# tijiang13/InstantAvatar

Hardware: AMD Instinct MI355X
Metric: novel_pose_render_frames_per_sec_512x512 (higher is better)
Workload: dtype f32; 1 GPU; render_image_fast 512x512, SNARF_NGP defaults (13 init bones, 128^2x32 skinning voxels, 16-level hash grid T=2^19, 64^3 occupancy rebuilt per frame with 5 probes, MAX_SAMPLES 256, MAX_BATCH 291600), synthetic SMPL-like body animated by the first 200 frames of data/animation/aist_demo.npz (animate.py:48-50 translation; tests/golden/aist_demo_200.npz); pose_track=aist_demo.npz[:200]

## Files before the change

### instantavatar_amd/csrc/ia_render.hip

```cpp
#include "ia_common.h"

int ia_launch_field(const float *x, int V, const int32_t *n_dev, const FieldDev &F, float *rgb,
                    float *sigma, hipStream_t s, uint16_t *acts);

__device__ __forceinline__ float clampf(float f, float a, float b) { return fmaxf(a, fminf(f, b)); }

__device__ __forceinline__ bool occ_test(const uint32_t *__restrict__ bits, int G, int nx, int ny, int nz) {
  const uint32_t idx = (uint32_t)((nx * G + ny) * G + nz);
  return (bits[idx >> 5] >> (idx & 31)) & 1u;
}

struct MarchRay {
  float ox, oy, oz, dx, dy, dz, cx, cy, cz, sx, sy, sz, far, dt;
};

__device__ __forceinline__ bool march_occupied(const MarchRay &r, const uint32_t *__restrict__ bits, int G,
                                               float t, float &x, float &y, float &z) {
  x = __builtin_fmaf(t, r.dx, r.ox); y = __builtin_fmaf(t, r.dy, r.oy); z = __builtin_fmaf(t, r.dz, r.oz);
  const float fx = (x - r.cx) * r.sx, fy = (y - r.cy) * r.sy, fz = (z - r.cz) * r.sz;
  const int nx = (int)clampf(fx, 0.0f, G - 1.0f);
  const int ny = (int)clampf(fy, 0.0f, G - 1.0f);
  const int nz = (int)clampf(fz, 0.0f, G - 1.0f);
  return occ_test(bits, G, nx, ny, nz);
}

__device__ __forceinline__ void march_skip(float &t, float dt, float lim) {
  if (dt > 0.f) {
    for (;;) {
      const float a = t + dt, b = a + dt, c = b + dt, d = c + dt, e = d + dt, f = e + dt, g = f + dt;
      if (!(g < lim)) break;
      t = g + dt;
    }
  }
  while (t < lim) t += dt;
}

__device__ __forceinline__ MarchRay load_ray(const float *__restrict__ o, const float *__restrict__ d,
                                             const float *__restrict__ fars, const float *__restrict__ step,
                                             size_t n, const float *aabb_mn, const float *aabb_mx, int G) {
  MarchRay r;
  r.ox = o[n * 3]; r.oy = o[n * 3 + 1]; r.oz = o[n * 3 + 2];
  r.dx = d[n * 3]; r.dy = d[n * 3 + 1]; r.dz = d[n * 3 + 2];
  r.cx = aabb_mn[0]; r.cy = aabb_mn[1]; r.cz = aabb_mn[2];
  r.sx = G / (aabb_mx[0] - aabb_mn[0]); r.sy = G / (aabb_mx[1] - aabb_mn[1]); r.sz = G / (aabb_mx[2] - aabb_mn[2]);
  r.far = fars[n]; r.dt = step[n];
  return r;
}

__global__ __launch_bounds__(256) void k_raymarch_test(const float *__restrict__ rays_o,
                                                       const float *__restrict__ rays_d, float *nears,
                                                       const float *__restrict__ fars,
                                                       const int64_t *__restrict__ alive, int n_alive,
                                                       const uint32_t *__restrict__ bits, OccDev occ,
                                                       const float *__restrict__ step, int N_steps,
                                                       float *__restrict__ pts, float *__restrict__ deltas,
                                                       float *__restrict__ depths) {
  const int i = blockIdx.x * blockDim.x + threadIdx.x;
  if (i >= n_alive) return;
  const size_t n = (size_t)alive[i];
  const MarchRay r = load_ray(rays_o, rays_d, fars, step, n, occ.mn, occ.mx, occ.G);
  int s = 0;
  float t = nears[n];
  while (t < r.far && s < N_steps) {
    float x, y, z;
    if (march_occupied(r, bits, occ.G, t, x, y, z)) {
      const size_t o = (size_t)i * N_steps + s;
      pts[o * 3] = x; pts[o * 3 + 1] = y; pts[o * 3 + 2] = z;
      deltas[o] = r.dt; depths[o] = t;
      s++;
    }
    t += r.dt;
  }
  for (; s < N_steps; s++) {
    const size_t o = (size_t)i * N_steps + s;
    pts[o * 3] = 0.f; pts[o * 3 + 1] = 0.f; pts[o * 3 + 2] = 0.f;
    deltas[o] = 0.f; depths[o] = 0.f;
  }
  nears[n] = t;
}

__global__ __launch_bounds__(256) void k_raymarch_train(const float *__restrict__ rays_o,
                                                        const float *__restrict__ rays_d,
                                                        const float *__restrict__ nears,
                                                        const float *__restrict__ fars, int n_rays,
                                                        const uint32_t *__restrict__ bits, OccDev occ,
                                                        const float *__restrict__ step, int N_steps,
                                                        float *__restrict__ depths) {
  const int n = blockIdx.x * blockDim.x + threadIdx.x;
  if (n >= n_rays) return;
  const MarchRay r = load_ray(rays_o, rays_d, fars, step, (size_t)n, occ.mn, occ.mx, occ.G);
  int s = 0;
  float t = nears[n];
  while (t < r.far && s < N_steps) {
    float x, y, z;
    if (march_occupied(r, bits, occ.G, t, x, y, z)) { depths[(size_t)n * N_steps + s] = t; s++; }
    t += r.dt;
  }
  for (; s < N_steps; s++) depths[(size_t)n * N_steps + s] = 0.f;
}

__device__ __forceinline__ void composite_step(float sg, float dl, float tdepth, const float *rgb3,
                                               float thresh, float &T, float &c0, float &c1, float &c2,
                                               float &dep) {
  const float tau = __expf(-sg * dl);
  const float alpha = 1.0f - tau;
  if (alpha < thresh) return;
  const float w = alpha * T;
  c0 += w * rgb3[0]; c1 += w * rgb3[1]; c2 += w * rgb3[2];
  dep += w * tdepth;
  T *= tau;
}

__global__ __launch_bounds__(256) void k_composite_test(const float *__restrict__ rgb,
                                                        const float *__restrict__ sigma,
                                                        const float *__restrict__ delta,
                                                        const float *__restrict__ depth,
                                                        const int64_t *__restrict__ alive, int n_alive,
                                                        int N_steps, float *color, float *depth_out,
                                                        float *nohit, float thresh) {
  const int i = blockIdx.x * blockDim.x + threadIdx.x;
  if (i >= n_alive) return;
  const size_t n = (size_t)alive[i];
  float T = nohit[n];
  float c0 = color[n * 3], c1 = color[n * 3 + 1], c2 = color[n * 3 + 2], dep = depth_out[n];
  int s = 0;
  while (s < N_steps && (double)T > 1e-4 && delta[(size_t)i * N_steps + s] > 0) {
    const size_t o = (size_t)i * N_steps + s;
    composite_step(sigma[o], delta[o], depth[o], rgb + o * 3, thresh, T, c0, c1, c2, dep);
    s++;
  }
  color[n * 3] = c0; color[n * 3 + 1] = c1; color[n * 3 + 2] = c2;
  depth_out[n] = dep;
  nohit[n] = T;
}

__device__ __forceinline__ void cand_max(const float *__restrict__ cand_rgb,
                                         const float *__restrict__ cand_sigma, int off, int cnt, int n_init,
                                         float fill, bool nan_to_num, float &sg, float *rgb3) {
  float best;
  int bi = -1;
  rgb3[0] = rgb3[1] = rgb3[2] = 0.f;
  if (cnt < n_init) best = fill; else best = -INFINITY;
  for (int c = 0; c < cnt; c++) {
    float s = cand_sigma[off + c];
    if (nan_to_num && !isfinite(s)) s = 0.f;
    if (s > best || (bi < 0 && cnt >= n_init && c == 0)) { best = s; bi = c; }
  }
  if (bi >= 0) {
#pragma unroll
    for (int k = 0; k < 3; k++) {
      float v = cand_rgb[(size_t)(off + bi) * 3 + k];
      if (nan_to_num && !isfinite(v)) v = 0.f;
      rgb3[k] = v;
    }
  }
  sg = best;
}

__global__ __launch_bounds__(256) void k_candidate_max(const float *__restrict__ cand_rgb,
                                                       const float *__restrict__ cand_sigma,
                                                       const int32_t *__restrict__ pt_off,
                                                       const uint8_t *__restrict__ pt_cnt, int P,
                                                       const int32_t *__restrict__ n_pts_dev, int n_init,
                                                       float fill, int nan_to_num, float *__restrict__ rgb,
                                                       float *__restrict__ sigma, float *__restrict__ dmax) {
  if (n_pts_dev) P = min(P, *n_pts_dev);
  const int p = blockIdx.x * blockDim.x + threadIdx.x;
  if (p >= P) return;
  float sg, c[3];
  cand_max(cand_rgb, cand_sigma, pt_off[p], pt_cnt[p], n_init, fill, nan_to_num != 0, sg, c);
  if (sigma) sigma[p] = sg;
  if (rgb) { rgb[(size_t)p * 3] = c[0]; rgb[(size_t)p * 3 + 1] = c[1]; rgb[(size_t)p * 3 + 2] = c[2]; }
  if (dmax) dmax[p] = fmaxf(dmax[p], sg);
}

struct OccWs {
  double sum;
  unsigned long long best;
  float thr;
  float pad;
};

__global__ __launch_bounds__(256) void k_occ_pool(const float *__restrict__ density, int G,
                                                  float *__restrict__ pooled, double *__restrict__ partial,
                                                  int32_t *__restrict__ parent, int32_t *__restrict__ count,
                                                  OccWs *__restrict__ ws, uint32_t *__restrict__ bits) {
  const int n = G * G * G;
  const int i = blockIdx.x * blockDim.x + threadIdx.x;
  if (i == 0) { ws->sum = 0.0; ws->best = 0ull; bits[n >> 5] = 1u; }
  float m = 0.f;
  if (i < n) {
    const int x = i / (G * G), y = i / G % G, z = i % G;
    m = -INFINITY;
    for (int a = -1; a <= 1; a++)
      for (int b = -1; b <= 1; b++)
        for (int c = -1; c <= 1; c++) {
          const int xx = x + a, yy = y + b, zz = z + c;
          if (xx < 0 || yy < 0 || zz < 0 || xx >= G || yy >= G || zz >= G) continue;
          const float f = 1.f - expf(0.01f * -density[(xx * G + yy) * G + zz]);
          m = (f > m || isnan(f)) ? f : m;
        }
    pooled[i] = m;
    parent[i] = i;
    count[i] = 0;
  }
  __shared__ double s_part[4];
  double v = (i < n) ? (double)m : 0.0;
#pragma unroll
  for (int o = 32; o > 0; o >>= 1) v += __shfl_xor(v, o, 64);
  if (ia_lane() == 0) s_part[threadIdx.x >> 6] = v;
  __syncthreads();
  if (threadIdx.x == 0) partial[blockIdx.x] = (s_part[0] + s_part[1]) + (s_part[2] + s_part[3]);
}

__device__ __forceinline__ float occ_threshold(const double *__restrict__ partial, int n_part, int n, double *s ) {
  double v = 0.0;
  for (int k = threadIdx.x; k < n_part; k += 256) v += partial[k];
  s[threadIdx.x] = v;
  __syncthreads();
  for (int o = 128; o > 0; o >>= 1) {
    if ((int)threadIdx.x < o) s[threadIdx.x] += s[threadIdx.x + o];
    __syncthreads();
  }
  const float mean = (float)(s[0] / (double)n);
  return mean > 0.01f ? 0.01f : mean;
}

__device__ __forceinline__ int uf_find(int32_t *parent, int i) {
  const int start = i;
  int p = __hip_atomic_load(&parent[i], __ATOMIC_RELAXED, __HIP_MEMORY_SCOPE_AGENT);
  while (p != i) { i = p; p = __hip_atomic_load(&parent[i], __ATOMIC_RELAXED, __HIP_MEMORY_SCOPE_AGENT); }
  if (start != i) atomicMax(&parent[start], i);
  return i;
}

__global__ __launch_bounds__(256) void k_occ_union(int G, const float *__restrict__ pooled,
                                                   const double *__restrict__ partial, int n_part, OccWs *ws,
                                                   int32_t *parent) {
  __shared__ double s_red[256];
  const int n = G * G * G;
  const float thr = occ_threshold(partial, n_part, n, s_red);
  const int i = blockIdx.x * blockDim.x + threadIdx.x;
  if (i == 0) { ws->thr = thr; ws->sum = s_red[0]; }
  if (i >= n || !(pooled[i] > thr)) return;
  const int x = i / (G * G), y = i / G % G, z = i % G;
  for (int a = 0; a <= 1; a++)
    for (int b = -1; b <= 1; b++)
      for (int c = -1; c <= 1; c++) {
        if (a == 0 && (b < 0 || (b == 0 && c <= 0))) continue;
        const int xx = x + a, yy = y + b, zz = z + c;
        if (xx >= G || yy < 0 || yy >= G || zz < 0 || zz >= G) continue;
        const int j = (xx * G + yy) * G + zz;
        if (!(pooled[j] > thr)) continue;
        int ra = i, rb = j;
        while (true) {
          ra = uf_find(parent, ra); rb = uf_find(parent, rb);
          if (ra == rb) break;
          if (ra > rb) { const int t = ra; ra = rb; rb = t; }
          const int old = atomicCAS(&parent[ra], ra, rb);
          if (old == ra) break;
        }
      }
}

__global__ __launch_bounds__(256) void k_occ_runs(const float *__restrict__ pooled, const double *__restrict__ partial,
                                                  int n_part, OccWs *ws, unsigned long long *__restrict__ colmask,
                                                  int32_t *__restrict__ parent) {
  __shared__ double s_red[256];
  constexpr int G = 64, n = G * G * G;
  const float thr = occ_threshold(partial, n_part, n, s_red);
  const int i = blockIdx.x * blockDim.x + threadIdx.x;
  if (i == 0) { ws->thr = thr; ws->sum = s_red[0]; }
  const int lane = i & 63;
  const bool occ = pooled[i] > thr;
  const unsigned long long m = __ballot(occ);
  if (lane == 0) colmask[i >> 6] = m;
  if (occ) {
    const unsigned long long above = ~m & ~((2ull << lane) - 1ull);
    const int end = (lane == 63 || above == 0ull) ? 63 : __ffsll((long long)above) - 2;
    parent[i] = (i & ~63) | end;
  }
}

__global__ __launch_bounds__(256) void k_occ_union_runs(const unsigned long long *__restrict__ colmask, int32_t *parent) {
  constexpr int G = 64;
  const int i = blockIdx.x * blockDim.x + threadIdx.x;
  const int col = i >> 6, z = i & 63;
  const unsigned long long m = colmask[col];
  const bool head = ((m >> z) & 1ull) && (z == 0 || !((m >> (z - 1)) & 1ull));
  if (!head) return;
  const unsigned long long above = ~m & ~((2ull << z) - 1ull);
  const int z1 = (z == 63 || above == 0ull) ? 63 : __ffsll((long long)above) - 2;
  const int lo = z > 0 ? z - 1 : 0, hi = z1 < 63 ? z1 + 1 : 63;
  const unsigned long long win = (hi == 63 ? ~0ull : ((2ull << hi) - 1ull)) & ~((1ull << lo) - 1ull);
  const int x = col >> 6, y = col & 63;
  const int self_end = (col << 6) | z1;
  const int nb[4][2] = {{0, 1}, {1, -1}, {1, 0}, {1, 1}};
#pragma unroll
  for (int k = 0; k < 4; k++) {
    const int xx = x + nb[k][0], yy = y + nb[k][1];
    if (xx >= G || yy < 0 || yy >= G) continue;
    const int ncol = xx * G + yy;
    const unsigned long long nm = colmask[ncol];
    unsigned long long t = nm & win;
    while (t) {
      const int b = __ffsll((long long)t) - 1;
      const unsigned long long nabove = ~nm & ~((2ull << b) - 1ull);
      const int e = (b == 63 || nabove == 0ull) ? 63 : __ffsll((long long)nabove) - 2;
      t &= ~((e == 63 ? ~0ull : ((2ull << e) - 1ull)));
      int ra = self_end, rb = (ncol << 6) | e;
      while (true) {
        ra = uf_find(parent, ra); rb = uf_find(parent, rb);
        if (ra == rb) break;
        if (ra > rb) { const int tt = ra; ra = rb; rb = tt; }
        const int old = atomicCAS(&parent[ra], ra, rb);
        if (old == ra) break;
      }
    }
  }
}

__global__ __launch_bounds__(256) void k_occ_count(int G, const float *__restrict__ pooled, const OccWs *__restrict__ ws,
                                                   int32_t *parent, int32_t *__restrict__ label, int32_t *count) {
  const int n = G * G * G;
  const int i = blockIdx.x * blockDim.x + threadIdx.x;
  if (i >= n) return;
  int l = -1;
  if (pooled[i] > ws->thr) l = uf_find(parent, i);
  label[i] = l;
  const unsigned long long m = __ballot(l >= 0);
  if (m) {
    const int first = __shfl(l, __ffsll((long long)m) - 1, 64);
    if (__all(l < 0 || l == first)) { if (ia_lane() == __ffsll((long long)m) - 1) atomicAdd(&count[first], __popcll(m)); }
    else if (l >= 0) atomicAdd(&count[l], 1);
  }
}

__global__ __launch_bounds__(256) void k_occ_best(int G, const int32_t *__restrict__ count, OccWs *ws) {
  const int n = G * G * G;
  const int i = blockIdx.x * blockDim.x + threadIdx.x;
  if (i >= n) return;
  const int c = count[i];
  if (c > 0) atomicMax(&ws->best, ((unsigned long long)c << 32) | (unsigned long long)(0xffffffffu - (uint32_t)i));
}

__global__ __launch_bounds__(256) void k_occ_final(int G, const int32_t *__restrict__ label,
                                                   const OccWs *__restrict__ ws, uint32_t *__restrict__ bits,
                                                   uint8_t *__restrict__ occ_bool) {
  const int n = G * G * G;
  const int i = blockIdx.x * blockDim.x + threadIdx.x;
  const unsigned long long best = ws->best;
  const int best_label = best ? (int)(0xffffffffu - (uint32_t)(best & 0xffffffffu)) : -2;
  const bool on = (i < n) && label[i] == best_label;
  if (i < n && occ_bool) occ_bool[i] = on;
  const unsigned long long m = __ballot(on);
  const int lane = ia_lane();
  if (i < n || (i - lane) < n) {
    if (lane == 0) bits[(i >> 5)] = (uint32_t)m;
    if (lane == 32) bits[(i >> 5)] = (uint32_t)(m >> 32);
  }
  if (on) {
    const int x = i / (G * G), y = i / G % G, z = i % G;
    if (x == 0 || y == 0 || z == 0 || x == G - 1 || y == G - 1 || z == G - 1) bits[n >> 5] = 0u;
  }
}

__global__ void k_occ_set_flag(uint32_t *bits, int n) { bits[n >> 5] = 1u; }

#define IA_OCC_TAIL_WORDS 8
__global__ __launch_bounds__(1024) void k_occ_bounds(uint32_t *__restrict__ bits, int G) {
  const int n_words = (G * G * G) >> 5;
  int mn[3] = {0x7fffffff, 0x7fffffff, 0x7fffffff}, mx[3] = {-1, -1, -1};
  if ((G & (G - 1)) == 0 && G >= 32) {
    const int sh = 31 - __clz(G);
    const uint4 *b4 = reinterpret_cast<const uint4 *>(bits);
    for (int q0 = threadIdx.x; q0 < n_words / 4; q0 += 2 * blockDim.x) {
      const int q1 = q0 + blockDim.x;
      const uint4 v0 = b4[q0];
      const uint4 v1 = q1 < n_words / 4 ? b4[q1] : make_uint4(0, 0, 0, 0);
      const uint32_t m[8] = {v0.x, v0.y, v0.z, v0.w, v1.x, v1.y, v1.z, v1.w};
#pragma unroll
      for (int k = 0; k < 8; k++) {
        if (!m[k]) continue;
        const int i = ((k < 4 ? q0 : q1) * 4 + (k & 3)) * 32;
        const int x = i >> (2 * sh), y = (i >> sh) & (G - 1), z0 = i & (G - 1);
        mn[0] = min(mn[0], x); mx[0] = max(mx[0], x);
        mn[1] = min(mn[1], y); mx[1] = max(mx[1], y);
        mn[2] = min(mn[2], z0 + __ffs((int)m[k]) - 1); mx[2] = max(mx[2], z0 + 31 - __clz((int)m[k]));
      }
    }
  } else {
    for (int w = threadIdx.x; w < n_words; w += blockDim.x) {
      uint32_t m = bits[w];
      while (m) {
        const int b = __ffs((int)m) - 1;
        m &= m - 1u;
        const int i = w * 32 + b;
        const int c[3] = {i / (G * G), i / G % G, i % G};
#pragma unroll
        for (int d = 0; d < 3; d++) { mn[d] = min(mn[d], c[d]); mx[d] = max(mx[d], c[d]); }
      }
    }
  }
  __shared__ int s_mn[16][3], s_mx[16][3];
#pragma unroll
  for (int d = 0; d < 3; d++) {
#pragma unroll
    for (int o = 32; o > 0; o >>= 1) { mn[d] = min(mn[d], __shfl_xor(mn[d], o, 64)); mx[d] = max(mx[d], __shfl_xor(mx[d], o, 64)); }
  }
  const int wv = threadIdx.x >> 6;
  if (ia_lane() == 0) {
#pragma unroll
    for (int d = 0; d < 3; d++) { s_mn[wv][d] = mn[d]; s_mx[wv][d] = mx[d]; }
  }
  __syncthreads();
  if (threadIdx.x < 3) {
    const int d = threadIdx.x;
    int a = 0x7fffffff, b = -1;
    for (int k = 0; k < (int)(blockDim.x >> 6); k++) { a = min(a, s_mn[k][d]); b = max(b, s_mx[k][d]); }
    bits[n_words + 1 + 2 * d] = (uint32_t)a;
    bits[n_words + 2 + 2 * d] = (uint32_t)b;
  }
}

__global__ __launch_bounds__(256) void k_occ_pack(const uint8_t *__restrict__ occ_bool, int n, int G,
                                                  uint32_t *__restrict__ bits) {
  const int i = blockIdx.x * blockDim.x + threadIdx.x;
  const bool on = (i < n) && occ_bool[i] != 0;
  if (on) {
    const int x = i / (G * G), y = i / G % G, z = i % G;
    if (x == 0 || y == 0 || z == 0 || x == G - 1 || y == G - 1 || z == G - 1) bits[n >> 5] = 0u;
  }
  const unsigned long long m = __ballot(on);
  const int lane = ia_lane();
  if ((i - lane) < n) {
    if (lane == 0) bits[(i >> 5)] = (uint32_t)m;
    if (lane == 32 && i < ((n + 31) / 32) * 32) bits[(i >> 5)] = (uint32_t)(m >> 32);
  }
}

__global__ void k_fill_f32(float *p, float v, int n) {
  const int i = blockIdx.x * blockDim.x + threadIdx.x;
  if (i < n) p[i] = v;
}
__global__ void k_fill_i32(int32_t *p, int32_t v, int n) {
  const int i = blockIdx.x * blockDim.x + threadIdx.x;
  if (i < n) p[i] = v;
}

__device__ __forceinline__ int ia_probe_cell(int c, int G) {
  if (G == 64) {
    int x = 0, y = 0, z = 0;
#pragma unroll
    for (int b = 0; b < 6; b++) {
      z |= ((c >> (3 * b)) & 1) << b;
      y |= ((c >> (3 * b + 1)) & 1) << b;
      x |= ((c >> (3 * b + 2)) & 1) << b;
    }
    return (x * G + y) * G + z;
  }
  const int x = c % G, y = c / G % G, z = c / (G * G);
  return (x * G + y) * G + z;
}

__global__ __launch_bounds__(256) void k_probe_points(const float *__restrict__ jitter, int G, int iters,
                                                      const float *__restrict__ aabb,
                                                      float *__restrict__ pts, int32_t *__restrict__ n_cand) {
  const int n = G * G * G;
  const int p = blockIdx.x * blockDim.x + threadIdx.x;
  if (p == 0) *n_cand = 0;
  if (p >= n * iters) return;
  const int it = p % iters, i = ia_probe_cell(p / iters, G);
  const int idx[3] = {i / (G * G), i / G % G, i % G};
#pragma unroll
  for (int d = 0; d < 3; d++) {
    const float c0 = (float)idx[d] / (float)G;
    const float c = c0 + jitter[((size_t)it * n + i) * 3 + d] / (float)G;
    pts[(size_t)p * 3 + d] = c * (aabb[3 + d] - aabb[d]) + aabb[d];
  }
}

__global__ __launch_bounds__(256) void k_transform_rays(const float *__restrict__ o, const float *__restrict__ d,
                                                        const float *__restrict__ w2s, int R,
                                                        float *__restrict__ o2, float *__restrict__ d2,
                                                        float *__restrict__ near, float *__restrict__ far) {
  const int i = blockIdx.x * blockDim.x + threadIdx.x;
  if (i >= R) return;
  const float ox = o[(size_t)i * 3], oy = o[(size_t)i * 3 + 1], oz = o[(size_t)i * 3 + 2];
  const float dx = d[(size_t)i * 3], dy = d[(size_t)i * 3 + 1], dz = d[(size_t)i * 3 + 2];
  float po[3], pd[3];
#pragma unroll
  for (int a = 0; a < 3; a++) {
    po[a] = ox * w2s[a * 4] + oy * w2s[a * 4 + 1] + oz * w2s[a * 4 + 2] + w2s[a * 4 + 3];
    pd[a] = dx * w2s[a * 4] + dy * w2s[a * 4 + 1] + dz * w2s[a * 4 + 2];
  }
  const float dist = sqrtf(po[0] * po[0] + po[1] * po[1] + po[2] * po[2]);
#pragma unroll
  for (int a = 0; a < 3; a++) { o2[(size_t)i * 3 + a] = po[a]; d2[(size_t)i * 3 + a] = pd[a]; }
  near[i] = dist - 1; far[i] = dist + 1;
}

#define IA_RENDER_MAX_ITERS 1024
struct RenderState {
  int32_t n_alive;
  int32_t n_samples;
  int32_t n_cand;
  int32_t k_before;
  int32_t iters;
  int32_t n_step;
  int32_t n_eff;
  int32_t pad;
};

__device__ __forceinline__ void render_schedule(const RenderState *st, int max_samples, int max_batch, int &na, int &ns) {
  na = st->n_alive;
  if (st->k_before >= max_samples) na = 0;
  ns = 0;
  if (na > 0) {
    ns = max_batch / na;
    ns = ns < max_samples ? ns : max_samples;
    ns = ns > 1 ? ns : 1;
  }
}

__global__ __launch_bounds__(256) void k_render_init_rays(int R, const float *__restrict__ near,
                                                          const float *__restrict__ far,
                                                          float *__restrict__ near_w, float *__restrict__ step,
                                                          float *__restrict__ color, float *__restrict__ depth,
                                                          float *__restrict__ nohit, float *__restrict__ counter,
                                                          int32_t *__restrict__ alive, int max_samples,
                                                          RenderState *st) {
  const int i = blockIdx.x * blockDim.x + threadIdx.x;
  for (int w = i; w < IA_RENDER_MAX_ITERS * (int)(sizeof(RenderState) / 4); w += gridDim.x * blockDim.x)
    reinterpret_cast<int32_t *>(st)[w] = (w == 0) ? R : 0;
  if (i >= R) return;
  near_w[i] = near[i];
  step[i] = (far[i] - near[i]) / max_samples;
  color[(size_t)i * 3] = 0.f; color[(size_t)i * 3 + 1] = 0.f; color[(size_t)i * 3 + 2] = 0.f;
  depth[i] = 0.f; nohit[i] = 1.f; counter[i] = 0.f;
  alive[i] = i;
}

#define IA_MARCH_LDS_WORDS (64 * 64 * 64 / 32)
template <bool LDS_BITS>
__global__ __launch_bounds__(256) void k_march_compact(
    const float *__restrict__ rays_o, const float *__restrict__ rays_d, float *near_w,
    const float *__restrict__ fars, const float *__restrict__ step, const int32_t *__restrict__ alive,
    RenderState *st, const uint32_t *bits_global, int G, const float *__restrict__ aabb,
    float *__restrict__ s_pts, float *__restrict__ s_t, int32_t *__restrict__ ray_off,
    int32_t *__restrict__ ray_cnt, float *__restrict__ counter, int sample_cap, int max_samples, int max_batch) {
  int n_alive, N_steps;
  render_schedule(st, max_samples, max_batch, n_alive, N_steps);
  const int i = blockIdx.x * blockDim.x + threadIdx.x;
  if (i == 0) {
    st->n_eff = n_alive; st->n_step = N_steps;
    st[1].k_before = st->k_before + N_steps;
    st[1].iters = st->iters + (n_alive > 0 ? 1 : 0);
  }
  if ((i - ia_lane()) >= n_alive) return;
  const bool live = i < n_alive;
  int cnt = 0;
  size_t n = 0;
  MarchRay r;
  float t0 = 0.f, t_end = 0.f, t_start = 0.f;
  if (live) {
    n = (size_t)alive[i];
    r = load_ray(rays_o, rays_d, fars, step, n, aabb, aabb + 3, G);
    t_start = near_w[n];
    t_end = t_start;
  }
  float t_lo = -INFINITY, t_hi = INFINITY;
  const uint32_t *tail = bits_global + ((G * G * G) >> 5);
  if (live && tail[0] == 1u) {
    const float lo[3] = {(float)(int)tail[1] - 0.05f, (float)(int)tail[3] - 0.05f, (float)(int)tail[5] - 0.05f};
    const float hi[3] = {(float)((int)tail[2] + 1) + 0.05f, (float)((int)tail[4] + 1) + 0.05f, (float)((int)tail[6] + 1) + 0.05f};
    const float A[3] = {(r.ox - r.cx) * r.sx, (r.oy - r.cy) * r.sy, (r.oz - r.cz) * r.sz};
    const float B[3] = {r.dx * r.sx, r.dy * r.sy, r.dz * r.sz};
    float a = -INFINITY, b = INFINITY;
#pragma unroll
    for (int c = 0; c < 3; c++) {
      if (!(lo[c] <= hi[c])) { a = INFINITY; b = -INFINITY; }
      else if (fabsf(B[c]) < 1e-12f) {
        if (!(A[c] >= lo[c] && A[c] <= hi[c])) { a = INFINITY; b = -INFINITY; }
      } else {
        const float t1 = (lo[c] - A[c]) / B[c], t2 = (hi[c] - A[c]) / B[c];
        a = fmaxf(a, fminf(t1, t2));
        b = fminf(b, fmaxf(t1, t2));
      }
    }
    if (a <= b) { t_lo = a - 2.f * r.dt; t_hi = b + 2.f * r.dt; }
    else { t_lo = INFINITY; t_hi = -INFINITY; }
  }
  __shared__ uint32_t s_bits[LDS_BITS ? IA_MARCH_LDS_WORDS : 1];
  __shared__ int s_any;
  if (LDS_BITS) {
    if (threadIdx.x == 0) s_any = 0;
    __syncthreads();
    if (__any(live && t_start < r.far && t_lo <= t_hi && t_start <= t_hi) && ia_lane() == 0) s_any = 1;
    __syncthreads();
    if (s_any) {
      const uint4 *src = reinterpret_cast<const uint4 *>(bits_global);
      uint4 *dst = reinterpret_cast<uint4 *>(s_bits);
      const int present = min(256, ((n_alive - (int)(blockIdx.x * blockDim.x)) + 63) & ~63);
      for (int w = threadIdx.x; w < IA_MARCH_LDS_WORDS / 4; w += present) dst[w] = src[w];
    }
    __syncthreads();
  }
  const uint32_t *bits = LDS_BITS ? s_bits : bits_global;
  if (live && r.dt > 0.f) {
    float t = t_start;
    t0 = t;
    bool found = false;
    march_skip(t, r.dt, fminf(r.far, t_lo));
    while (t < r.far && cnt < N_steps && t <= t_hi) {
      const float t1 = t + r.dt, t2 = t1 + r.dt, t3 = t2 + r.dt;
      float x, y, z;
      const bool o0 = march_occupied(r, bits, G, t, x, y, z), o1 = march_occupied(r, bits, G, t1, x, y, z);
      const bool o2 = march_occupied(r, bits, G, t2, x, y, z), o3 = march_occupied(r, bits, G, t3, x, y, z);
      if (o0) { if (!found) { found = true; t0 = t; } cnt++; }
      t = t1;
      if (!(t < r.far && cnt < N_steps)) break;
      if (o1) { if (!found) { found = true; t0 = t; } cnt++; }
      t = t2;
      if (!(t < r.far && cnt < N_steps)) break;
      if (o2) { if (!found) { found = true; t0 = t; } cnt++; }
      t = t3;
      if (!(t < r.far && cnt < N_steps)) break;
      if (o3) { if (!found) { found = true; t0 = t; } cnt++; }
      t = t3 + r.dt;
    }
    if (cnt < N_steps) march_skip(t, r.dt, r.far);
    t_end = t;
  }
  int total;
  const int excl = ia_wave_excl_scan(cnt, total);
  int base = 0;
  if (ia_lane() == 0 && total > 0) base = atomicAdd(&st->n_samples, total);
  base = __shfl(base, 0, 64) + excl;
  if (!live) return;
  ray_off[i] = base;
  ray_cnt[i] = cnt;
  counter[n] += (float)cnt;
  near_w[n] = t_end;
  int s = 0;
  float t = t0;
  auto emit = [&](float tt, float x, float y, float z) {
    const int o = base + s;
    if (o < sample_cap) { s_pts[(size_t)o * 3] = x; s_pts[(size_t)o * 3 + 1] = y; s_pts[(size_t)o * 3 + 2] = z; s_t[o] = tt; }
    s++;
  };
  while (t < r.far && s < cnt) {
    const float t1 = t + r.dt, t2 = t1 + r.dt, t3 = t2 + r.dt;
    float x0, y0, z0, x1, y1, z1, x2, y2, z2, x3, y3, z3;
    const bool o0 = march_occupied(r, bits, G, t, x0, y0, z0), o1 = march_occupied(r, bits, G, t1, x1, y1, z1);
    const bool o2 = march_occupied(r, bits, G, t2, x2, y2, z2), o3 = march_occupied(r, bits, G, t3, x3, y3, z3);
    if (o0) emit(t, x0, y0, z0);
    if (!(t1 < r.far && s < cnt)) break;
    if (o1) emit(t1, x1, y1, z1);
    if (!(t2 < r.far && s < cnt)) break;
    if (o2) emit(t2, x2, y2, z2);
    if (!(t3 < r.far && s < cnt)) break;
    if (o3) emit(t3, x3, y3, z3);
    t = t3 + r.dt;
  }
}

__global__ __launch_bounds__(256) void k_composite_compact(
    const int32_t *__restrict__ alive, int32_t *__restrict__ alive_next, RenderState *st,
    const int32_t *__restrict__ ray_off, const int32_t *__restrict__ ray_cnt,
    const float *__restrict__ s_t, const float *__restrict__ step, const int32_t *__restrict__ pt_off,
    const uint8_t *__restrict__ pt_cnt, const float *__restrict__ cand_rgb,
    const float *__restrict__ cand_sigma, int n_init, float *color, float *depth, float *nohit,
    float thresh) {
  const int n_alive = st->n_eff;
  const int i = blockIdx.x * blockDim.x + threadIdx.x;
  if ((i - ia_lane()) >= n_alive) return;
  const int N_steps = st->n_step;
  bool keep = false;
  int n = 0;
  if (i < n_alive) {
    n = alive[i];
    const int off = ray_off[i], cnt = ray_cnt[i];
    const float dt = step[n];
    float T = nohit[n];
    float c0 = color[(size_t)n * 3], c1 = color[(size_t)n * 3 + 1], c2 = color[(size_t)n * 3 + 2];
    float dep = depth[n];
    int s = 0;
    while (s < cnt && (double)T > 1e-4 && dt > 0) {
      const int m = min(4, cnt - s);
      int po[4], pc[4], bi[4];
      float tz[4], best[4], rgb[4][3];
#pragma unroll
      for (int j = 0; j < 4; j++) {
        const int q = off + s + (j < m ? j : 0);
        po[j] = pt_off[q]; pc[j] = j < m ? (int)pt_cnt[q] : 0; tz[j] = s_t[q];
        best[j] = pc[j] < n_init ? 0.f : -INFINITY;
        bi[j] = -1;
      }
      const int cmax = max(max(pc[0], pc[1]), max(pc[2], pc[3]));
      for (int c = 0; c < cmax; c++) {
        float sv[4];
#pragma unroll
        for (int j = 0; j < 4; j++) sv[j] = c < pc[j] ? cand_sigma[po[j] + c] : 0.f;
#pragma unroll
        for (int j = 0; j < 4; j++) {
          if (c < pc[j]) {
            float v = sv[j];
            if (!isfinite(v)) v = 0.f;
            if (v > best[j] || (bi[j] < 0 && pc[j] >= n_init && c == 0)) { best[j] = v; bi[j] = c; }
          }
        }
      }
#pragma unroll
      for (int j = 0; j < 4; j++) {
#pragma unroll
        for (int k = 0; k < 3; k++) {
          float v = bi[j] >= 0 ? cand_rgb[(size_t)(po[j] + bi[j]) * 3 + k] : 0.f;
          if (!isfinite(v)) v = 0.f;
          rgb[j][k] = v;
        }
      }
#pragma unroll
      for (int j = 0; j < 4; j++) {
        if (j < m && (double)T > 1e-4) composite_step(best[j], dt, tz[j], rgb[j], thresh, T, c0, c1, c2, dep);
      }
      s += m;
    }
    color[(size_t)n * 3] = c0; color[(size_t)n * 3 + 1] = c1; color[(size_t)n * 3 + 2] = c2;
    depth[n] = dep;
    nohit[n] = T;
    const bool last_filled = (cnt == N_steps) && (s_t[off + cnt - 1] > 0.f);
    keep = ((double)T > 1e-4) && last_filled;
  }
  const unsigned long long m = __ballot(keep);
  const int total = __popcll(m);
  int base = 0;
  if (ia_lane() == 0 && total > 0) base = atomicAdd(&st[1].n_alive, total);
  base = __shfl(base, 0, 64);
  if (keep) alive_next[base + __popcll(m & ((1ull << ia_lane()) - 1ull))] = n;
}

__global__ __launch_bounds__(256) void k_render_finalize(int R, const float *__restrict__ color,
                                                         const float *__restrict__ depth,
                                                         const float *__restrict__ nohit,
                                                         const float *__restrict__ counter,
                                                         const float *__restrict__ bg, const RenderState *st_end,
                                                         int max_samples, int32_t *__restrict__ n_alive_out,
                                                         float *__restrict__ rgb_out, float *__restrict__ depth_out,
                                                         float *__restrict__ alpha_out,
                                                         float *__restrict__ counter_out) {
  const int i = blockIdx.x * blockDim.x + threadIdx.x;
  if (i == 0 && n_alive_out) {
    int na = st_end->n_alive;
    if (st_end->k_before >= max_samples) na = 0;
    n_alive_out[0] = na; n_alive_out[1] = st_end->iters;
  }
  if (i >= R) return;
  const float T = nohit[i];
#pragma unroll
  for (int c = 0; c < 3; c++)
    rgb_out[(size_t)i * 3 + c] = color[(size_t)i * 3 + c] + T * (bg ? bg[(size_t)i * 3 + c] : 1.0f);
  depth_out[i] = depth[i];
  alpha_out[i] = 1.f - T;
  counter_out[i] = counter[i];
}

static OccDev make_occ(const ia_occ_grid *o) {
  OccDev d;
  d.G = o->G;
  for (int i = 0; i < 3; i++) { d.mn[i] = o->aabb_min[i]; d.mx[i] = o->aabb_max[i]; }
  return d;
}

extern "C" int ia_raymarch_test(const float *rays_o, const float *rays_d, float *nears, const float *fars,
                                const int64_t *alive, int n_alive, const uint32_t *occ_bits,
                                const ia_occ_grid *occ, const float *step_size, int N_steps, float *pts,
                                float *deltas, float *depths, void *stream) {
  IA_CHECK_ARG(n_alive >= 0 && N_steps > 0, "ia_raymarch_test: bad sizes");
  if (n_alive == 0) return IA_OK;
  IA_CHECK_ARG(rays_o && rays_d && nears && fars && alive && occ_bits && occ && step_size && pts && deltas && depths,
               "ia_raymarch_test: null pointer");
  hipLaunchKernelGGL(k_raymarch_test, dim3(ia_div_up(n_alive, 256)), dim3(256), 0, (hipStream_t)stream, rays_o,
                     rays_d, nears, fars, alive, n_alive, occ_bits, make_occ(occ), step_size, N_steps, pts, deltas,
                     depths);
  IA_LAUNCH_CHECK("k_raymarch_test");
  return IA_OK;
}

extern "C" int ia_raymarch_train(const float *rays_o, const float *rays_d, const float *nears,
                                 const float *fars, int n_rays, const uint32_t *occ_bits,
                                 const ia_occ_grid *occ, const float *step_size, int N_steps, float *depths,
                                 void *stream) {
  IA_CHECK_ARG(n_rays >= 0 && N_steps > 0, "ia_raymarch_train: bad sizes");
  if (n_rays == 0) return IA_OK;
  IA_CHECK_ARG(rays_o && rays_d && nears && fars && occ_bits && occ && step_size && depths,
               "ia_raymarch_train: null pointer");
  hipLaunchKernelGGL(k_raymarch_train, dim3(ia_div_up(n_rays, 256)), dim3(256), 0, (hipStream_t)stream, rays_o,
                     rays_d, nears, fars, n_rays, occ_bits, make_occ(occ), step_size, N_steps, depths);
  IA_LAUNCH_CHECK("k_raymarch_train");
  return IA_OK;
}

extern "C" int ia_composite_test(const float *rgb, const float *sigma, const float *delta, const float *depth,
                                 const int64_t *alive, int n_alive, int N_steps, float *color,
                                 float *depth_out, float *no_hit, float thresh, void *stream) {
  IA_CHECK_ARG(n_alive >= 0 && N_steps > 0, "ia_composite_test: bad sizes");
  if (n_alive == 0) return IA_OK;
  IA_CHECK_ARG(rgb && sigma && delta && depth && alive && color && depth_out && no_hit,
               "ia_composite_test: null pointer");
  hipLaunchKernelGGL(k_composite_test, dim3(ia_div_up(n_alive, 256)), dim3(256), 0, (hipStream_t)stream, rgb,
                     sigma, delta, depth, alive, n_alive, N_steps, color, depth_out, no_hit, thresh);
  IA_LAUNCH_CHECK("k_composite_test");
  return IA_OK;
}

extern "C" int ia_candidate_max(const float *cand_rgb, const float *cand_sigma, const int32_t *pt_off,
                                const uint8_t *pt_cnt, int P, const int32_t *n_pts_dev, int n_init, float fill,
                                int nan_to_num, float *rgb, float *sigma, void *stream) {
  IA_CHECK_ARG(P >= 0, "ia_candidate_max: P < 0");
  if (P == 0) return IA_OK;
  IA_CHECK_ARG(cand_rgb && cand_sigma && pt_off && pt_cnt, "ia_candidate_max: null pointer");
  hipLaunchKernelGGL(k_candidate_max, dim3(ia_div_up(P, 256)), dim3(256), 0, (hipStream_t)stream, cand_rgb,
                     cand_sigma, pt_off, pt_cnt, P, n_pts_dev, n_init, fill, nan_to_num, rgb, sigma,
                     (float *)nullptr);
  IA_LAUNCH_CHECK("k_candidate_max");
  return IA_OK;
}

extern "C" size_t ia_occupancy_workspace_bytes(int G) {
  const size_t n = (size_t)G * G * G;
  return ia_align(sizeof(OccWs)) + 5 * ia_align(n * 4) + ia_align((n / 256 + 1) * 8) + 1024;
}

extern "C" int ia_occupancy_from_density(const float *density, int G, uint32_t *occ_bits, uint8_t *occ_bool,
                                         void *ws, size_t ws_bytes, void *stream) {
  IA_CHECK_ARG(density && occ_bits && ws, "ia_occupancy_from_density: null pointer");
  IA_CHECK_ARG(G >= 4 && G <= 256 && (G * G * G) % 64 == 0, "ia_occupancy_from_density: unsupported G=%d", G);
  if (ws_bytes < ia_occupancy_workspace_bytes(G)) return ia_set_error(IA_ERR_WORKSPACE, "ia_occupancy_from_density: workspace too small");
  hipStream_t s = (hipStream_t)stream;
  const int n = G * G * G;
  WsCarver w(ws, ws_bytes);
  OccWs *ow = w.take<OccWs>(1);
  float *pooled = w.take<float>(n);
  int32_t *parent = w.take<int32_t>(n);
  int32_t *label = w.take<int32_t>(n);
  int32_t *count = w.take<int32_t>(n);
  float *fval = w.take<float>(n);
  double *partial = w.take<double>(ia_div_up(n, 256));
  const dim3 grid(ia_div_up(n, 256)), blk(256);
  const int n_part = ia_div_up(n, 256);
  hipLaunchKernelGGL(k_occ_pool, grid, blk, 0, s, density, G, pooled, partial, parent, count, ow, occ_bits);
  if (G == 64) {
    unsigned long long *colmask = reinterpret_cast<unsigned long long *>(fval);
    hipLaunchKernelGGL(k_occ_runs, grid, blk, 0, s, pooled, partial, n_part, ow, colmask, parent);
    hipLaunchKernelGGL(k_occ_union_runs, grid, blk, 0, s, colmask, parent);
  } else {
    hipLaunchKernelGGL(k_occ_union, grid, blk, 0, s, G, pooled, partial, n_part, ow, parent);
  }
  hipLaunchKernelGGL(k_occ_count, grid, blk, 0, s, G, pooled, ow, parent, label, count);
  hipLaunchKernelGGL(k_occ_best, grid, blk, 0, s, G, count, ow);
  hipLaunchKernelGGL(k_occ_final, grid, blk, 0, s, G, label, ow, occ_bits, occ_bool);
  hipLaunchKernelGGL(k_occ_bounds, dim3(1), dim3(1024), 0, s, occ_bits, G);
  IA_LAUNCH_CHECK("occupancy_from_density");
  return IA_OK;
}

extern "C" int ia_occupancy_pack(const uint8_t *occ_bool, int G, uint32_t *occ_bits, void *stream) {
  IA_CHECK_ARG(occ_bool && occ_bits && G > 0 && (G * G * G) % 64 == 0, "ia_occupancy_pack: bad arguments");
  const int n = G * G * G;
  hipLaunchKernelGGL(k_occ_set_flag, dim3(1), dim3(1), 0, (hipStream_t)stream, occ_bits, n);
  hipLaunchKernelGGL(k_occ_pack, dim3(ia_div_up(n, 256)), dim3(256), 0, (hipStream_t)stream, occ_bool, n, G, occ_bits);
  hipLaunchKernelGGL(k_occ_bounds, dim3(1), dim3(1024), 0, (hipStream_t)stream, occ_bits, G);
  IA_LAUNCH_CHECK("k_occ_pack");
  return IA_OK;
}

struct QueryWs {
  int32_t *n_cand; int32_t *pt_off; uint8_t *pt_cnt; float *cand_xc; float *cand_rgb; float *cand_sigma;
  int cand_cap;
};
static size_t query_ws_bytes(int P, int n_init) {
  const size_t cap = (size_t)P * n_init;
  return ia_align(256) + ia_align((size_t)P * 4) + ia_align((size_t)P) + 2 * ia_align(cap * 12) + ia_align(cap * 4);
}
static QueryWs carve_query(WsCarver &w, int P, int n_init) {
  QueryWs q;
  const size_t cap = (size_t)P * n_init;
  q.n_cand = w.take<int32_t>(64);
  q.pt_off = w.take<int32_t>(P);
  q.pt_cnt = w.take<uint8_t>(P);
  q.cand_xc = w.take<float>(cap * 3);
  q.cand_rgb = w.take<float>(cap * 3);
  q.cand_sigma = w.take<float>(cap);
  q.cand_cap = (int)cap;
  return q;
}

extern "C" size_t ia_query_workspace_bytes(int P, int n_init) { return query_ws_bytes(P, n_init) + 1024; }

static int query_impl(const float *pts, int P, const int32_t *n_pts_dev, const float *voxel_J, const float *tfs,
                      const int32_t *bone_ids, int n_init, const ia_snarf_grid *grid, const FieldDev &F,
                      const QueryWs &q, hipStream_t s, int zero_counter = 1) {
  int rc = ia_snarf_search_compact(pts, P, n_pts_dev, voxel_J, tfs, bone_ids, n_init, grid, 1e-5f, 1e-1f,
                                   q.cand_xc, q.cand_cap, q.pt_off, q.pt_cnt, q.n_cand, zero_counter, s);
  if (rc) return rc;
  return ia_launch_field(q.cand_xc, q.cand_cap, q.n_cand, F, q.cand_rgb, q.cand_sigma, s, nullptr);
}

extern "C" int ia_deform_query(const float *pts, int P, const int32_t *n_pts_dev, const float *voxel_J,
                               const float *tfs, const int32_t *bone_ids, int n_init, const ia_snarf_grid *grid,
                               const ia_field *field, float *rgb, float *sigma, float *dmax, void *ws,
                               size_t ws_bytes, void *stream) {
  IA_CHECK_ARG(P >= 0, "ia_deform_query: P < 0");
  if (P == 0) return IA_OK;
  IA_CHECK_ARG(pts && ws, "ia_deform_query: null pointer");
  if (ws_bytes < ia_query_workspace_bytes(P, n_init)) return ia_set_error(IA_ERR_WORKSPACE, "ia_deform_query: workspace too small");
  FieldDev F;
  int rc = ia_make_field_dev(field, &F);
  IA_CHECK_ARG(rc == 0, "ia_deform_query: bad field descriptor (%d)", rc);
  WsCarver w(ws, ws_bytes);
  QueryWs q = carve_query(w, P, n_init);
  hipStream_t s = (hipStream_t)stream;
  rc = query_impl(pts, P, n_pts_dev, voxel_J, tfs, bone_ids, n_init, grid, F, q, s);
  if (rc) return rc;
  hipLaunchKernelGGL(k_candidate_max, dim3(ia_div_up(P, 256)), dim3(256), 0, s, q.cand_rgb, q.cand_sigma, q.pt_off,
                     q.pt_cnt, P, n_pts_dev, n_init, 0.f, 1, rgb, sigma, dmax);
  IA_LAUNCH_CHECK("k_candidate_max");
  return IA_OK;
}

extern "C" size_t ia_density_init_workspace_bytes(int G, int n_init) {
  const int n = G * G * G;
  return ia_align((size_t)n * 12) + query_ws_bytes(n, n_init) + ia_occupancy_workspace_bytes(G) + 4096;
}

extern "C" size_t ia_density_init_workspace_bytes_batched(int G, int n_init, int iters) {
  const size_t n = (size_t)G * G * G * (size_t)(iters > 0 ? iters : 1);
  if (n * (size_t)n_init > 0x7fffffffu) return 0;
  return ia_align(n * 12) + query_ws_bytes((int)n, n_init) + ia_occupancy_workspace_bytes(G) + 4096;
}

__global__ __launch_bounds__(256) void k_probe_max(const float *__restrict__ cand_rgb,
                                                   const float *__restrict__ cand_sigma,
                                                   const int32_t *__restrict__ pt_off,
                                                   const uint8_t *__restrict__ pt_cnt, int n, int G, int iters, int n_init,
                                                   float *__restrict__ density, int accumulate) {
  const int c = blockIdx.x * blockDim.x + threadIdx.x;
  if (c >= n) return;
  const int i = ia_probe_cell(c, G);
  float m = accumulate ? density[i] : 0.f;
  for (int it = 0; it < iters; it++) {
    const size_t p = (size_t)c * iters + it;
    float sg, col[3];
    cand_max(cand_rgb, cand_sigma, pt_off[p], pt_cnt[p], n_init, 0.f, true, sg, col);
    m = fmaxf(m, sg);
  }
  density[i] = m;
}

extern "C" int ia_density_grid_init(const float *jitter, int iters, int G, const float *aabb,
                                    const float *voxel_J, const float *tfs, const int32_t *bone_ids, int n_init,
                                    const ia_snarf_grid *grid, const ia_field *field, float *density,
                                    uint32_t *occ_bits, uint8_t *occ_bool, void *ws, size_t ws_bytes,
                                    void *stream) {
  IA_CHECK_ARG(jitter && aabb && density && occ_bits && ws && iters >= 1, "ia_density_grid_init: bad arguments");
  if (ws_bytes < ia_density_init_workspace_bytes(G, n_init)) return ia_set_error(IA_ERR_WORKSPACE, "ia_density_grid_init: workspace too small");
  FieldDev F;
// ... 502 lines not shown
```

Before: 662.1 frames/s.

## Stage only occupied x-slab of occupancy bits into LDS and skip empty-ray work

The march kernel previously copied the whole 64^3 occupancy bitfield (32 KB) into shared memory per block. It now copies only the x-rows covered by the occupied bounding box (capped at 42 rows) and looks up bits through a slab accessor that treats out-of-slab cells as empty. It falls back to global-memory lookups when the box is larger. The trimmed path also skips marching for rays that miss the box, drops the trailing skip loop, and writes counter and near only when needed. This cuts LDS footprint and copy traffic, which can raise occupancy, at the cost of extra index math per lookup and more branching.

```diff
diff --git a/instantavatar_amd/csrc/ia_render.hip b/instantavatar_amd/csrc/ia_render.hip
--- a/instantavatar_amd/csrc/ia_render.hip
+++ b/instantavatar_amd/csrc/ia_render.hip
@@ -14,14 +14,37 @@
   float ox, oy, oz, dx, dy, dz, cx, cy, cz, sx, sy, sz, far, dt;
 };
 
-__device__ __forceinline__ bool march_occupied(const MarchRay &r, const uint32_t *__restrict__ bits, int G,
-                                               float t, float &x, float &y, float &z) {
+struct OccGrid {
+  const uint32_t *__restrict__ bits;
+  int G;
+  __device__ __forceinline__ bool operator()(int nx, int ny, int nz) const { return occ_test(bits, G, nx, ny, nz); }
+};
+struct OccSlab {
+  const uint32_t *words;
+  uint32_t w_lo, n_words;
+  __device__ __forceinline__ bool operator()(int nx, int ny, int nz) const {
+    const uint32_t idx = (uint32_t)((nx * 64 + ny) * 64 + nz);
+    const uint32_t w = (idx >> 5) - w_lo;
+    const bool in = w < n_words;
+    const uint32_t v = words[in ? w : 0u];
+    return ((v >> (idx & 31)) & (in ? 1u : 0u)) != 0u;
+  }
+};
+
+template <class Occ>
+__device__ __forceinline__ bool march_occupied_in(const MarchRay &r, const Occ &occ, int G,
+                                                  float t, float &x, float &y, float &z) {
   x = __builtin_fmaf(t, r.dx, r.ox); y = __builtin_fmaf(t, r.dy, r.oy); z = __builtin_fmaf(t, r.dz, r.oz);
   const float fx = (x - r.cx) * r.sx, fy = (y - r.cy) * r.sy, fz = (z - r.cz) * r.sz;
   const int nx = (int)clampf(fx, 0.0f, G - 1.0f);
   const int ny = (int)clampf(fy, 0.0f, G - 1.0f);
   const int nz = (int)clampf(fz, 0.0f, G - 1.0f);
-  return occ_test(bits, G, nx, ny, nz);
+  return occ(nx, ny, nz);
+}
+
+__device__ __forceinline__ bool march_occupied(const MarchRay &r, const uint32_t *__restrict__ bits, int G,
+                                               float t, float &x, float &y, float &z) {
+  return march_occupied_in(r, OccGrid{bits, G}, G, t, x, y, z);
 }
 
 __device__ __forceinline__ void march_skip(float &t, float dt, float lim) {
@@ -541,7 +564,79 @@
   alive[i] = i;
 }
 
-#define IA_MARCH_LDS_WORDS (64 * 64 * 64 / 32)
+#define IA_MARCH_SLAB_ROWS 42
+template <bool TRIM, class Occ>
+__device__ __forceinline__ void march_two_pass(const Occ &occ, bool live, const MarchRay &r, size_t n, int i, float t_start,
+                                               float t_lo, float t_hi, int N_steps, int G, RenderState *st, float *near_w,
+                                               float *__restrict__ s_pts, float *__restrict__ s_t, int32_t *__restrict__ ray_off,
+                                               int32_t *__restrict__ ray_cnt, float *__restrict__ counter, int sample_cap) {
+  int cnt = 0;
+  float t0 = 0.f, t_end = t_start;
+  bool march = live && r.dt > 0.f;
+  if (TRIM) march = march && t_start < r.far && t_lo <= t_hi && t_start <= t_hi && t_lo < r.far;
+  if (march) {
+    float t = t_start;
+    t0 = t;
+    bool found = false;
+    march_skip(t, r.dt, fminf(r.far, t_lo));
+    while (t < r.far && cnt < N_steps && t <= t_hi) {
+      const float t1 = t + r.dt, t2 = t1 + r.dt, t3 = t2 + r.dt;
+      float x, y, z;
+      const bool o0 = march_occupied_in(r, occ, G, t, x, y, z), o1 = march_occupied_in(r, occ, G, t1, x, y, z);
+      const bool o2 = march_occupied_in(r, occ, G, t2, x, y, z), o3 = march_occupied_in(r, occ, G, t3, x, y, z);
+      if (o0) { if (!found) { found = true; t0 = t; } cnt++; }
+      t = t1;
+      if (!(t < r.far && cnt < N_steps)) break;
+      if (o1) { if (!found) { found = true; t0 = t; } cnt++; }
+      t = t2;
+      if (!(t < r.far && cnt < N_steps)) break;
+      if (o2) { if (!found) { found = true; t0 = t; } cnt++; }
+      t = t3;
+      if (!(t < r.far && cnt < N_steps)) break;
+      if (o3) { if (!found) { found = true; t0 = t; } cnt++; }
+      t = t3 + r.dt;
+    }
+    if (!TRIM && cnt < N_steps) march_skip(t, r.dt, r.far);
+    t_end = t;
+  }
+  int total;
+  const int excl = ia_wave_excl_scan(cnt, total);
+  int base = 0;
+  if (ia_lane() == 0 && total > 0) base = atomicAdd(&st->n_samples, total);
+  base = __shfl(base, 0, 64) + excl;
+  if (!live) return;
+  ray_off[i] = base;
+  ray_cnt[i] = cnt;
+  if (TRIM) {
+    if (cnt > 0) counter[n] += (float)cnt;
+    if (cnt == N_steps) near_w[n] = t_end;
+  } else {
+    counter[n] += (float)cnt;
+    near_w[n] = t_end;
+  }
+  int s = 0;
+  float t = t0;
+  auto emit = [&](float tt, float x, float y, float z) {
+    const int o = base + s;
+    if (o < sample_cap) { s_pts[(size_t)o * 3] = x; s_pts[(size_t)o * 3 + 1] = y; s_pts[(size_t)o * 3 + 2] = z; s_t[o] = tt; }
+    s++;
+  };
+  while (t < r.far && s < cnt) {
+    const float t1 = t + r.dt, t2 = t1 + r.dt, t3 = t2 + r.dt;
+    float x0, y0, z0, x1, y1, z1, x2, y2, z2, x3, y3, z3;
+    const bool o0 = march_occupied_in(r, occ, G, t, x0, y0, z0), o1 = march_occupied_in(r, occ, G, t1, x1, y1, z1);
+    const bool o2 = march_occupied_in(r, occ, G, t2, x2, y2, z2), o3 = march_occupied_in(r, occ, G, t3, x3, y3, z3);
+    if (o0) emit(t, x0, y0, z0);
+    if (!(t1 < r.far && s < cnt)) break;
+    if (o1) emit(t1, x1, y1, z1);
+    if (!(t2 < r.far && s < cnt)) break;
+    if (o2) emit(t2, x2, y2, z2);
+    if (!(t3 < r.far && s < cnt)) break;
+    if (o3) emit(t3, x3, y3, z3);
+    t = t3 + r.dt;
+  }
+}
+
 template <bool LDS_BITS>
 __global__ __launch_bounds__(256) void k_march_compact(
     const float *__restrict__ rays_o, const float *__restrict__ rays_d, float *near_w,
@@ -559,15 +654,13 @@
   }
   if ((i - ia_lane()) >= n_alive) return;
   const bool live = i < n_alive;
-  int cnt = 0;
   size_t n = 0;
   MarchRay r;
-  float t0 = 0.f, t_end = 0.f, t_start = 0.f;
+  float t_start = 0.f;
   if (live) {
     n = (size_t)alive[i];
     r = load_ray(rays_o, rays_d, fars, step, n, aabb, aabb + 3, G);
     t_start = near_w[n];
-    t_end = t_start;
   }
   float t_lo = -INFINITY, t_hi = INFINITY;
   const uint32_t *tail = bits_global + ((G * G * G) >> 5);
@@ -591,78 +684,34 @@
     if (a <= b) { t_lo = a - 2.f * r.dt; t_hi = b + 2.f * r.dt; }
     else { t_lo = INFINITY; t_hi = -INFINITY; }
   }
-  __shared__ uint32_t s_bits[LDS_BITS ? IA_MARCH_LDS_WORDS : 1];
+  if (!LDS_BITS) {
+    march_two_pass<false>(OccGrid{bits_global, G}, live, r, n, i, t_start, t_lo, t_hi, N_steps, G, st, near_w, s_pts, s_t, ray_off,
+                          ray_cnt, counter, sample_cap);
+    return;
+  }
+  const int x_lo = (int)tail[1], x_hi = (int)tail[2];
+  const bool none = x_lo > x_hi;
+  const int rows = none ? 0 : x_hi - x_lo + 1;
+  const bool slab = tail[0] == 1u && (none || (x_lo >= 0 && x_hi < G && rows <= IA_MARCH_SLAB_ROWS));
+  if (!slab) {
+    march_two_pass<true>(OccGrid{bits_global, G}, live, r, n, i, t_start, t_lo, t_hi, N_steps, G, st, near_w, s_pts, s_t, ray_off,
+                         ray_cnt, counter, sample_cap);
+    return;
+  }
+  __shared__ uint4 s_rows[LDS_BITS ? IA_MARCH_SLAB_ROWS * 32 : 1];
   __shared__ int s_any;
-  if (LDS_BITS) {
-    if (threadIdx.x == 0) s_any = 0;
-    __syncthreads();
-    if (__any(live && t_start < r.far && t_lo <= t_hi && t_start <= t_hi) && ia_lane() == 0) s_any = 1;
-    __syncthreads();
-    if (s_any) {
-      const uint4 *src = reinterpret_cast<const uint4 *>(bits_global);
-      uint4 *dst = reinterpret_cast<uint4 *>(s_bits);
-      const int present = min(256, ((n_alive - (int)(blockIdx.x * blockDim.x)) + 63) & ~63);
-      for (int w = threadIdx.x; w < IA_MARCH_LDS_WORDS / 4; w += present) dst[w] = src[w];
-    }
-    __syncthreads();
-  }
-  const uint32_t *bits = LDS_BITS ? s_bits : bits_global;
-  if (live && r.dt > 0.f) {
-    float t = t_start;
-    t0 = t;
-    bool found = false;
-    march_skip(t, r.dt, fminf(r.far, t_lo));
-    while (t < r.far && cnt < N_steps && t <= t_hi) {
-      const float t1 = t + r.dt, t2 = t1 + r.dt, t3 = t2 + r.dt;
-      float x, y, z;
-      const bool o0 = march_occupied(r, bits, G, t, x, y, z), o1 = march_occupied(r, bits, G, t1, x, y, z);
-      const bool o2 = march_occupied(r, bits, G, t2, x, y, z), o3 = march_occupied(r, bits, G, t3, x, y, z);
-      if (o0) { if (!found) { found = true; t0 = t; } cnt++; }
-      t = t1;
-      if (!(t < r.far && cnt < N_steps)) break;
-      if (o1) { if (!found) { found = true; t0 = t; } cnt++; }
-      t = t2;
-      if (!(t < r.far && cnt < N_steps)) break;
-      if (o2) { if (!found) { found = true; t0 = t; } cnt++; }
-      t = t3;
-      if (!(t < r.far && cnt < N_steps)) break;
-      if (o3) { if (!found) { found = true; t0 = t; } cnt++; }
-      t = t3 + r.dt;
-    }
-    if (cnt < N_steps) march_skip(t, r.dt, r.far);
-    t_end = t;
-  }
-  int total;
-  const int excl = ia_wave_excl_scan(cnt, total);
-  int base = 0;
-  if (ia_lane() == 0 && total > 0) base = atomicAdd(&st->n_samples, total);
-  base = __shfl(base, 0, 64) + excl;
-  if (!live) return;
-  ray_off[i] = base;
-  ray_cnt[i] = cnt;
-  counter[n] += (float)cnt;
-  near_w[n] = t_end;
-  int s = 0;
-  float t = t0;
-  auto emit = [&](float tt, float x, float y, float z) {
-    const int o = base + s;
-    if (o < sample_cap) { s_pts[(size_t)o * 3] = x; s_pts[(size_t)o * 3 + 1] = y; s_pts[(size_t)o * 3 + 2] = z; s_t[o] = tt; }
-    s++;
-  };
-  while (t < r.far && s < cnt) {
-    const float t1 = t + r.dt, t2 = t1 + r.dt, t3 = t2 + r.dt;
-    float x0, y0, z0, x1, y1, z1, x2, y2, z2, x3, y3, z3;
-    const bool o0 = march_occupied(r, bits, G, t, x0, y0, z0), o1 = march_occupied(r, bits, G, t1, x1, y1, z1);
-    const bool o2 = march_occupied(r, bits, G, t2, x2, y2, z2), o3 = march_occupied(r, bits, G, t3, x3, y3, z3);
-    if (o0) emit(t, x0, y0, z0);
-    if (!(t1 < r.far && s < cnt)) break;
-    if (o1) emit(t1, x1, y1, z1);
-    if (!(t2 < r.far && s < cnt)) break;
-    if (o2) emit(t2, x2, y2, z2);
-    if (!(t3 < r.far && s < cnt)) break;
-    if (o3) emit(t3, x3, y3, z3);
-    t = t3 + r.dt;
-  }
+  if (threadIdx.x == 0) s_any = 0;
+  __syncthreads();
+  if (__any(live && r.dt > 0.f && t_start < r.far && t_lo <= t_hi && t_start <= t_hi && t_lo < r.far) && ia_lane() == 0) s_any = 1;
+  __syncthreads();
+  if (s_any) {
+    const uint4 *src = reinterpret_cast<const uint4 *>(bits_global) + x_lo * 32;
+    const int present = min(256, ((n_alive - (int)(blockIdx.x * blockDim.x)) + 63) & ~63);
+    for (int w = threadIdx.x; w < rows * 32; w += present) s_rows[w] = src[w];
+  }
+  __syncthreads();
+  march_two_pass<true>(OccSlab{reinterpret_cast<const uint32_t *>(s_rows), (uint32_t)x_lo * 128u, (uint32_t)rows * 128u}, live, r, n, i,
+                       t_start, t_lo, t_hi, N_steps, G, st, near_w, s_pts, s_t, ray_off, ray_cnt, counter, sample_cap);
 }
 
 __global__ __launch_bounds__(256) void k_composite_compact(
```

After: 663.9 frames/s, median of 6. No clear change (+0.3%).
